# ivanalberico/End-To-End-Self-Supervised-SLAM

Hardware: AMD Instinct MI355X
Metric: online refinement steps/sec @640x480, seq_len=60 (higher is better)
Workload: dtype f32

## Files before the change

end-to-end-self-supervised-slam_amd/csrc/conv.hip:

```cpp
#include <cassert>
#include <type_traits>

#include "e2e_common.h"

typedef float f4v __attribute__((ext_vector_type(4)));
typedef float f16v __attribute__((ext_vector_type(16)));

#define CBK 16

enum { ACT_NONE = 0, ACT_RELU = 1, ACT_ELU = 2, ACT_DISP = 3 };

struct ConvArgs {
    const float* src0;
    const float* src1;
    const float* w;
    const float* scale;
    const float* shift;
    const float* res;
    float* out;
    int B, Hs, Ws;
    int Cin, C1, up;
    int Hd, Wd;
    int Ncols, ldw;
    int KH, KW, stride, pad, pad_mode;
// ... 2046 lines not shown

__global__ __launch_bounds__(256) void k_gather_adjoint(const float* __restrict__ dxp, int B, int Hs, int Ws, int Cin, int C1, int up,
                                                        int pp, float* __restrict__ d0, float* __restrict__ d1, int acc0, int acc1,
                                                        const float* __restrict__ x0, int act0, const float* __restrict__ x1, int act1) {
    const int Hp = Hs + 2 * pp, Wp = Ws + 2 * pp, C2 = Cin - C1, Hl = Hs / up, Wl = Ws / up;
    const int64_t n0 = (int64_t)B * Hl * Wl * C1, n1 = (int64_t)B * Hs * Ws * C2;
    for (int64_t i = (int64_t)blockIdx.x * 256 + threadIdx.x; i < n0 + n1; i += (int64_t)gridDim.x * 256) {
        const bool first = i < n0;
        int64_t t = first ? i : i - n0;
        const int Cx = first ? C1 : C2, Hx = first ? Hl : Hs, Wx = first ? Wl : Ws, u = first ? up : 1;
        const int c = (int)(t % Cx); t /= Cx;
        const int x = (int)(t % Wx); t /= Wx;
        const int y = (int)(t % Hx); t /= Hx;
        const int b = (int)t;
        const int cc = first ? c : C1 + c;
        float s = 0.f;
        for (int dy = 0; dy < u; ++dy)
            for (int dx = 0; dx < u; ++dx) {
                const int fy = y * u + dy, fx = x * u + dx;
                int ys[3] = {fy + pp, -1, -1}, xs[3] = {fx + pp, -1, -1};
                if (pp) {
                    if (fy == 1) ys[1] = 0;
                    if (fy == Hs - 2) ys[2] = Hp - 1;
                    if (fx == 1) xs[1] = 0;
                    if (fx == Ws - 2) xs[2] = Wp - 1;
                }
                for (int iy = 0; iy < 3; ++iy)
                    for (int ix = 0; ix < 3; ++ix)
                        if (ys[iy] >= 0 && xs[ix] >= 0) s += dxp[(((int64_t)b * Hp + ys[iy]) * Wp + xs[ix]) * Cin + cc];
            }
        float* d = first ? d0 + i : d1 + (i - n0);
        const int acc = first ? acc0 : acc1;
        if (first ? act0 : act1) s *= act_deriv(first ? x0[i] : x1[i - n0], first ? act0 : act1);
        *d = acc ? *d + s : s;
    }
}

__global__ __launch_bounds__(256) void k_gather_adjoint4(const float* __restrict__ dxp, int B, int Hs, int Ws, int Cin, int C1, int up,
                                                         int pp, float* __restrict__ d0, float* __restrict__ d1, int acc0, int acc1,
                                                         const float* __restrict__ x0, int act0, const float* __restrict__ x1, int act1) {
    const int Hp = Hs + 2 * pp, Wp = Ws + 2 * pp, C2 = Cin - C1, Hl = Hs / up, Wl = Ws / up;
    const unsigned q0 = (unsigned)B * Hl * Wl * (C1 >> 2), q1 = (unsigned)B * Hs * Ws * (C2 >> 2);
    for (unsigned i = blockIdx.x * 256u + threadIdx.x; i < q0 + q1; i += gridDim.x * 256u) {
        const bool first = i < q0;
        unsigned t = first ? i : i - q0;
        const unsigned Cq = (unsigned)(first ? C1 : C2) >> 2, Hx = first ? Hl : Hs, Wx = first ? Wl : Ws;
        const int u = first ? up : 1;
        const unsigned cq = t % Cq; t /= Cq;
        const unsigned x = t % Wx; t /= Wx;
        const unsigned y = t % Hx;
        const unsigned b = t / Hx;
        const int cc = (first ? 0 : C1) + (int)cq * 4;
        f4v s = {0.f, 0.f, 0.f, 0.f};
        for (int dy = 0; dy < u; ++dy)
            for (int dx = 0; dx < u; ++dx) {
                const int fy = (int)y * u + dy, fx = (int)x * u + dx;
                int ys[3] = {fy + pp, -1, -1}, xs[3] = {fx + pp, -1, -1};
                if (pp) {
                    if (fy == 1) ys[1] = 0;
                    if (fy == Hs - 2) ys[2] = Hp - 1;
                    if (fx == 1) xs[1] = 0;
                    if (fx == Ws - 2) xs[2] = Wp - 1;
                }
#pragma unroll
                for (int iy = 0; iy < 3; ++iy)
#pragma unroll
                    for (int ix = 0; ix < 3; ++ix)
                        if (ys[iy] >= 0 && xs[ix] >= 0) s += *(const f4v*)(dxp + (((int64_t)b * Hp + ys[iy]) * Wp + xs[ix]) * Cin + cc);
            }
        const int64_t e = (int64_t)(first ? i : i - q0) * 4;
        const int act = first ? act0 : act1;
        if (act) {
            const f4v xv = *(const f4v*)((first ? x0 : x1) + e);
#pragma unroll
            for (int k = 0; k < 4; ++k) s[k] *= act_deriv(xv[k], act);
        }
        f4v* d = (f4v*)((first ? d0 : d1) + e);
        if (first ? acc0 : acc1) s += *d;
        *d = s;
    }
}

#define HC 16
__global__ __launch_bounds__(256) void k_head_fwd(const float* __restrict__ x, const float* __restrict__ w ,
                                                  const float* __restrict__ bias, float* __restrict__ y, int B, int H, int W, int act) {
    __shared__ float sw[9 * HC];
    for (int i = threadIdx.x; i < 9 * HC; i += 256) {
        const int ci = i / 9, tap = i - ci * 9;
        sw[tap * HC + ci] = w[i];
    }
    __syncthreads();
    const int64_t N = (int64_t)B * H * W;
    const int q = threadIdx.x & 3;
    for (int64_t n0 = (int64_t)blockIdx.x * 64; n0 < N; n0 += (int64_t)gridDim.x * 64) {
        const int64_t n = n0 + (threadIdx.x >> 2);
        const bool on = n < N;
        const int64_t nn = on ? n : N - 1;
        const int b = (int)(nn / ((int64_t)H * W));
        const int r = (int)(nn - (int64_t)b * H * W), h = r / W, ww = r - h * W;
        float acc = 0.f;
#pragma unroll
        for (int kh = 0; kh < 3; ++kh)
#pragma unroll
            for (int kw = 0; kw < 3; ++kw) {
                const int ys = reflect1(h + kh - 1, H), xs = reflect1(ww + kw - 1, W);
                const f4v v = *(const f4v*)(x + (((int64_t)b * H + ys) * W + xs) * HC + q * 4);
                const float* wt = &sw[(kh * 3 + kw) * HC + q * 4];
                acc = fmaf(v[0], wt[0], fmaf(v[1], wt[1], fmaf(v[2], wt[2], fmaf(v[3], wt[3], acc))));
            }
        acc += __shfl_xor(acc, 1, 64);
        acc += __shfl_xor(acc, 2, 64);
        if (on && q == 0) y[n] = apply_act(acc + (bias ? bias[0] : 0.f), act);
    }
}

__global__ __launch_bounds__(256) void k_head_bwd_data(const float* __restrict__ dz, const float* __restrict__ w, float* __restrict__ dx,
                                                       int B, int H, int W, const float* __restrict__ xin, int dact) {
    __shared__ float sw[9 * HC];
    for (int i = threadIdx.x; i < 9 * HC; i += 256) {
        const int ci = i / 9, tap = i - ci * 9;
        sw[tap * HC + ci] = w[i];
    }
    __syncthreads();
    const int64_t N = (int64_t)B * H * W;
    const int cq = threadIdx.x & 3;
    for (int64_t n = (int64_t)blockIdx.x * 64 + (threadIdx.x >> 2); n < N; n += (int64_t)gridDim.x * 64) {
        const int b = (int)(n / ((int64_t)H * W));
        const int r = (int)(n - (int64_t)b * H * W), h = r / W, ww = r - h * W;
        f4v acc = {0.f, 0.f, 0.f, 0.f};
        const int ry = (h == 1) ? 0 : ((h == H - 2) ? H + 1 : -100);
        const int rx = (ww == 1) ? 0 : ((ww == W - 2) ? W + 1 : -100);
        const float* gz = dz + (int64_t)b * H * W;
#pragma unroll
        for (int kh = 0; kh < 3; ++kh)
#pragma unroll
            for (int kw = 0; kw < 3; ++kw) {
                const float* wt = &sw[(kh * 3 + kw) * HC + cq * 4];
                const int qy0 = h - kh + 1, qx0 = ww - kw + 1, qy1 = ry - kh, qx1 = rx - kw;
                const bool y0 = qy0 >= 0 && qy0 < H, x0 = qx0 >= 0 && qx0 < W, y1 = qy1 >= 0 && qy1 < H, x1 = qx1 >= 0 && qx1 < W;
                float g = (y0 && x0) ? gz[(int64_t)qy0 * W + qx0] : 0.f;
                if (y1 | x1) {
                    if (y0 && x1) g += gz[(int64_t)qy0 * W + qx1];
                    if (y1 && x0) g += gz[(int64_t)qy1 * W + qx0];
                    if (y1 && x1) g += gz[(int64_t)qy1 * W + qx1];
                }
#pragma unroll
                for (int c = 0; c < 4; ++c) acc[c] = fmaf(g, wt[c], acc[c]);
            }
        if (dact) {
            const f4v xv = *(const f4v*)(xin + n * HC + cq * 4);
#pragma unroll
            for (int e = 0; e < 4; ++e) acc[e] *= act_deriv(xv[e], dact);
        }
        *(f4v*)(dx + n * HC + cq * 4) = acc;
    }
}

__global__ __launch_bounds__(256) void k_head_bwd_weight(const float* __restrict__ dz, const float* __restrict__ x, float* __restrict__ partials,
                                                         int B, int H, int W) {
    __shared__ float red[4][9 * HC + 1];
    const int64_t N = (int64_t)B * H * W;
    const int lane = threadIdx.x & 63, wave = threadIdx.x >> 6, cq = threadIdx.x & 3, ps = threadIdx.x >> 2;
    const int64_t per = (N + gridDim.x - 1) / gridDim.x;
    const int64_t n0 = (int64_t)blockIdx.x * per, n1 = (n0 + per < N) ? n0 + per : N;
    float acc[36];
#pragma unroll
    for (int k = 0; k < 36; ++k) acc[k] = 0.f;
    float sb = 0.f;
    for (int64_t n = n0 + ps; n < n1; n += 64) {
        const float g = dz[n];
        const int b = (int)(n / ((int64_t)H * W));
        const int r = (int)(n - (int64_t)b * H * W), h = r / W, ww = r - h * W;
#pragma unroll
        for (int kh = 0; kh < 3; ++kh)
#pragma unroll
            for (int kw = 0; kw < 3; ++kw) {
                const int ys = reflect1(h + kh - 1, H), xs = reflect1(ww + kw - 1, W);
                const f4v v = *(const f4v*)(x + (((int64_t)b * H + ys) * W + xs) * HC + cq * 4);
#pragma unroll
                for (int c = 0; c < 4; ++c) acc[(kh * 3 + kw) * 4 + c] = fmaf(g, v[c], acc[(kh * 3 + kw) * 4 + c]);
            }
        sb += g;
    }
#pragma unroll
    for (int k = 0; k < 36; ++k) {
        float v = acc[k];
#pragma unroll
        for (int o = 4; o < 64; o <<= 1) v += __shfl_xor(v, o, 64);
        acc[k] = v;
    }
#pragma unroll
    for (int o = 4; o < 64; o <<= 1) sb += __shfl_xor(sb, o, 64);
    if (lane < 4) {
#pragma unroll
        for (int t = 0; t < 9; ++t)
#pragma unroll
            for (int c = 0; c < 4; ++c) red[wave][t * HC + lane * 4 + c] = acc[t * 4 + c];
        if (lane == 0) red[wave][9 * HC] = sb;
    }
    __syncthreads();
    if (threadIdx.x < 9 * HC + 1)
        partials[(int64_t)blockIdx.x * (9 * HC + 1) + threadIdx.x] = ((red[0][threadIdx.x] + red[1][threadIdx.x]) + red[2][threadIdx.x]) + red[3][threadIdx.x];
}

__global__ __launch_bounds__(256) void k_head_wreduce(const float* __restrict__ partials, int nparts, float* __restrict__ dw, float* __restrict__ dbias) {
    __shared__ float red[4];
    const int col = blockIdx.x;
    float s = 0.f;
    for (int i = threadIdx.x; i < nparts; i += 256) s += partials[(int64_t)i * (9 * HC + 1) + col];
    const float t = block_sum(s, red);
    if (threadIdx.x == 0) {
        if (col == 9 * HC) { if (dbias) dbias[0] = t; }
        else { const int tap = col / HC, ci = col - tap * HC; dw[ci * 9 + tap] = t; }
    }
}

static inline int egrid(int64_t n) { int64_t g = (n + 255) / 256; return (int)(g < 1 ? 1 : (g > 4096 ? 4096 : g)); }

struct GemmCfg { int bm, bn, S; };
#define WGRAD_TARGET 1024

#define CONV_TILE_SHAPES(X)                                                                                      \
    X(64, 64, 2, 2, 1, 1, 32) X(128, 64, 2, 2, 2, 1, 32) X(128, 128, 2, 2, 2, 2, 16) X(128, 32, 4, 1, 1, 1, 32) \
    X(32, 128, 1, 4, 1, 1, 32) X(32, 64, 1, 2, 1, 1, 32) X(64, 32, 2, 1, 1, 1, 32) X(32, 32, 1, 1, 1, 1, 32)
static int tile_max_cb(int bm, int bn) {
#define X(BM, BN, WM, WN, TM, TN, MAXCB) if (bm == BM && bn == BN) return MAXCB;
    CONV_TILE_SHAPES(X)
// ... 333 lines not shown
    if (rc != E2E_OK) return rc;
    if (!done) launch_gemm<true>(a, 4, workspace, force, (hipStream_t)stream);
    E2E_LAUNCH_CHECK("e2e_conv2d_bwd_data");
    return E2E_OK;
}

int e2e_conv2d_bwd_data(const float* dz, const float* w_bwd, int ld_bwd, float* dxp, int B, int Hs, int Ws, int Cin, int Cout,
                        int Ho, int Wo, int KH, int KW, int stride, int pad, int pad_mode, float* workspace, void* stream) {
    GEOM_BWD_DATA(g);
    return bwd_data_impl(BwdDataOps{dz, w_bwd, ld_bwd, dxp, 0, nullptr, 0, nullptr}, g, workspace, stream);
}

int e2e_conv2d_bwd_data_acc(const float* dz, const float* w_bwd, int ld_bwd, float* dxp, int B, int Hs, int Ws, int Cin, int Cout,
                            int Ho, int Wo, int KH, int KW, int stride, int pad, int pad_mode, int accumulate, float* workspace,
                            void* stream) {
    GEOM_BWD_DATA(g);
    return bwd_data_impl(BwdDataOps{dz, w_bwd, ld_bwd, dxp, accumulate, nullptr, 0, nullptr}, g, workspace, stream);
}

int e2e_conv2d_bwd_data_fused(const float* da, const float* w_bwd, int ld_bwd, float* dxp, int B, int Hs, int Ws, int Cin, int Cout,
                              int Ho, int Wo, int KH, int KW, int stride, int pad, int pad_mode, int accumulate, const float* x_in,
                              int in_act, const float* pre_add, float* workspace, void* stream) {
    GEOM_BWD_DATA(g);
    return bwd_data_impl(BwdDataOps{da, w_bwd, ld_bwd, dxp, accumulate, x_in, in_act, pre_add}, g, workspace, stream);
}

int e2e_conv2d_bwd_data_fused_tuned(const float* da, const float* w_bwd, int ld_bwd, float* dxp, int B, int Hs, int Ws, int Cin, int Cout,
                                    int Ho, int Wo, int KH, int KW, int stride, int pad, int pad_mode, int accumulate, const float* x_in,
                                    int in_act, const float* pre_add, float* workspace, int tile_m, int tile_n, int ksplit, void* stream) {
    E2E_REQUIRE(tuning_ok(tile_m, tile_n, ksplit), E2E_ERR_ARG, "e2e_conv2d_bwd_data_fused_tuned: unsupported decomposition %d x %d / %d", tile_m, tile_n, ksplit);
    GEOM_BWD_DATA(g);
    return bwd_data_impl(BwdDataOps{da, w_bwd, ld_bwd, dxp, accumulate, x_in, in_act, pre_add}, g, workspace, stream, GemmCfg{tile_m, tile_n, ksplit});
}

struct GatherAdjoint { const float* dxp; int B, Hs, Ws, Cin, C1, up, padded; float *d0, *d1; int acc0, acc1; const float* x0; int act0; const float* x1; int act1; };
static void launch_gather_adjoint(const GatherAdjoint& q, hipStream_t st) {
    const int64_t n = (int64_t)q.B * (q.Hs / q.up) * (q.Ws / q.up) * q.C1 + (int64_t)q.B * q.Hs * q.Ws * (q.Cin - q.C1);
    if (q.Cin % 4 == 0 && q.C1 % 4 == 0 && n < (1ll << 31))
        hipLaunchKernelGGL(k_gather_adjoint4, dim3(egrid(n / 4)), dim3(256), 0, st, q.dxp, q.B, q.Hs, q.Ws, q.Cin, q.C1, q.up, q.padded ? 1 : 0, q.d0, q.d1, q.acc0, q.acc1,
                           q.x0, q.act0, q.x1, q.act1);
    else
        hipLaunchKernelGGL(k_gather_adjoint, dim3(egrid(n)), dim3(256), 0, st, q.dxp, q.B, q.Hs, q.Ws, q.Cin, q.C1, q.up, q.padded ? 1 : 0, q.d0, q.d1, q.acc0, q.acc1,
                           q.x0, q.act0, q.x1, q.act1);
}

int e2e_conv2d_gather_adjoint(const float* dxp, int B, int Hs, int Ws, int Cin, int C1, int up, int padded, float* d_src0,
                              float* d_src1, int accumulate0, int accumulate1, void* stream) {
    E2E_REQUIRE(dxp && d_src0 && B > 0 && Cin > 0 && C1 > 0 && C1 <= Cin && (C1 == Cin || d_src1) && (up == 1 || up == 2), E2E_ERR_ARG,
                "e2e_conv2d_gather_adjoint: bad argument");
    launch_gather_adjoint(GatherAdjoint{dxp, B, Hs, Ws, Cin, C1, up, padded, d_src0, d_src1, accumulate0, accumulate1, nullptr, 0, nullptr, 0}, (hipStream_t)stream);
    E2E_LAUNCH_CHECK("e2e_conv2d_gather_adjoint");
    return E2E_OK;
}

int e2e_conv2d_gather_adjoint_act(const float* dxp, int B, int Hs, int Ws, int Cin, int C1, int up, int padded, float* d_src0, float* d_src1,
                                  int accumulate0, int accumulate1, const float* src0, int act0, const float* src1, int act1, void* stream) {
    E2E_REQUIRE(dxp && d_src0 && B > 0 && Cin > 0 && C1 > 0 && C1 <= Cin && (C1 == Cin || d_src1) && (up == 1 || up == 2), E2E_ERR_ARG,
                "e2e_conv2d_gather_adjoint_act: bad argument");
    E2E_REQUIRE((act0 == 0 || src0) && (act1 == 0 || src1) && act0 >= 0 && act0 <= 2 && act1 >= 0 && act1 <= 2, E2E_ERR_ARG,
                "e2e_conv2d_gather_adjoint_act: an activation derivative needs the activation's output");
    launch_gather_adjoint(GatherAdjoint{dxp, B, Hs, Ws, Cin, C1, up, padded, d_src0, d_src1, accumulate0, accumulate1, src0, act0, src1, act1}, (hipStream_t)stream);
    E2E_LAUNCH_CHECK("e2e_conv2d_gather_adjoint_act");
    return E2E_OK;
}

int e2e_conv2d_act_bwd(const float* dy, const float* y, const float* scale, float* dz, int64_t n, int C, int act, void* stream) {
    E2E_REQUIRE(dy && y && dz && n > 0 && C > 0 && act >= 0 && act <= 3, E2E_ERR_ARG, "e2e_conv2d_act_bwd: bad argument");
    hipLaunchKernelGGL(k_act_bwd, dim3(egrid(n)), dim3(256), 0, (hipStream_t)stream, dy, y, scale, dz, n, C, act, 0);
    E2E_LAUNCH_CHECK("e2e_conv2d_act_bwd");
    return E2E_OK;
}

int e2e_conv2d_act_bwd_acc(const float* dy, const float* y, const float* scale, float* dz, int64_t n, int C, int act, int accumulate,
                           void* stream) {
    E2E_REQUIRE(dy && y && dz && n > 0 && C > 0 && act >= 0 && act <= 3, E2E_ERR_ARG, "e2e_conv2d_act_bwd_acc: bad argument");
    hipLaunchKernelGGL(k_act_bwd, dim3(egrid(n)), dim3(256), 0, (hipStream_t)stream, dy, y, scale, dz, n, C, act, accumulate);
    E2E_LAUNCH_CHECK("e2e_conv2d_act_bwd_acc");
    return E2E_OK;
}

#define HEAD_PARTS 2048
int e2e_head_fwd(const float* x, const float* w, const float* bias, float* y, int B, int H, int W, int Cin, int act, void* stream) {
    E2E_REQUIRE(x && w && y && B > 0 && H >= 2 && W >= 2 && Cin == HC, E2E_ERR_ARG, "e2e_head_fwd: bad argument (the head takes %d channels)", HC);
    hipLaunchKernelGGL(k_head_fwd, dim3(egrid((int64_t)B * H * W * 4)), dim3(256), 0, (hipStream_t)stream, x, w, bias, y, B, H, W, act);
    E2E_LAUNCH_CHECK("e2e_head_fwd");
    return E2E_OK;
}
int64_t e2e_head_workspace_floats(void) { return (int64_t)HEAD_PARTS * (9 * HC + 1); }
int e2e_head_bwd_act(const float* dz, const float* x, const float* w, float* dx, float* dw, float* dbias, float* workspace, int B, int H,
                     int W, int Cin, int in_act, void* stream) {
    E2E_REQUIRE(dz && x && w && workspace && B > 0 && H >= 2 && W >= 2 && Cin == HC && in_act >= 0 && in_act <= 2, E2E_ERR_ARG, "e2e_head_bwd: bad argument");
    E2E_REQUIRE((int64_t)B * H * W * HC < (1ll << 31), E2E_ERR_ARG, "e2e_head_bwd: activation too large for 32-bit element offsets");
    hipStream_t st = (hipStream_t)stream;
    if (dx) hipLaunchKernelGGL(k_head_bwd_data, dim3(egrid((int64_t)B * H * W * 4)), dim3(256), 0, st, dz, w, dx, B, H, W, x, in_act);
    if (dw) {
        hipLaunchKernelGGL(k_head_bwd_weight, dim3(HEAD_PARTS), dim3(256), 0, st, dz, x, workspace, B, H, W);
        hipLaunchKernelGGL(k_head_wreduce, dim3(9 * HC + 1), dim3(256), 0, st, workspace, HEAD_PARTS, dw, dbias);
    }
    E2E_LAUNCH_CHECK("e2e_head_bwd");
    return E2E_OK;
}

int e2e_head_bwd(const float* dz, const float* x, const float* w, float* dx, float* dw, float* dbias, float* workspace, int B, int H,
                 int W, int Cin, void* stream) {
    return e2e_head_bwd_act(dz, x, w, dx, dw, dbias, workspace, B, H, W, Cin, 0, stream);
}

enum WgradPath { WP_STEM, WP_THIN, WP_TAPS, WP_GEMM16, WP_GEMM_LEAN, WP_GEMM, WP_COUNT };
struct WgradPlan { WgradPath path; bool open; int64_t S; int Mpad, Npad, tm, tn, nxg, ny, tiles_x, ptx, pty, nchunks, cps; };
#define TAP_TARGET 640
static WgradPlan wgrad_plan(WgradPath path, const ConvGeom& g, int has_bias, bool tuned, int wg_target) {
    const int B = g.B, Ho = g.Ho, Wo = g.Wo, Cin = g.Cin, Cout = g.Cout, KH = g.KH, KW = g.KW;
    WgradPlan p{path};
    if (path == WP_STEM) {
        if (tuned || !(KH == 7 && KW == 7 && Cin == 3 && Cout == 64)) return p;
        p.nxg = ((Wo + 31) / 32 + 1) / 2; p.ny = (Ho + 3) / 4;
        p.S = (int64_t)B * p.ny * p.nxg; p.Mpad = 64; p.Npad = 148;
    } else if (path == WP_THIN) {
        if (tuned || !(KH == 3 && KW == 3 && ((Cout == 16 && (Cin == 16 || Cin == 32)) || (Cout == 32 && Cin == 96)))) return p;
        const int txt = (Wo + 63) / 64;
        p.ny = (Ho + 3) / 4;
        const int64_t total = (int64_t)B * p.ny * txt * (Cin / 16);
        p.tiles_x = 1;
        while (total / p.tiles_x > 1400 && p.tiles_x < txt) ++p.tiles_x;
        p.nxg = (txt + p.tiles_x - 1) / p.tiles_x;
        p.S = (int64_t)B * p.ny * p.nxg; p.Mpad = Cout; p.Npad = (9 * Cin + (has_bias ? 1 : 0) + 3) / 4 * 4;
    } else if (path == WP_TAPS) {
        if (tuned || !(KH == 3 && KW == 3 && Cin % 32 == 0 && Cout % 32 == 0)) return p;
        p.ptx = (Wo + 7) / 8; p.pty = (Ho + 7) / 8;
        p.nchunks = B * p.ptx * p.pty;
        const int tiles = (Cin / 32) * (Cout / 32);
        int S = (TAP_TARGET + tiles - 1) / tiles;
        if (S > p.nchunks) S = p.nchunks;
        if (S < 1) S = 1;
        p.cps = (p.nchunks + S - 1) / S;
        p.S = (p.nchunks + p.cps - 1) / p.cps; p.Mpad = Cout; p.Npad = (9 * Cin + (has_bias ? 1 : 0) + 3) / 4 * 4;
    } else {
        const bool use16 = path == WP_GEMM16;
        if (use16 && Cout != 16) return p;
        const int Ng = KH * KW * Cin + (has_bias ? 1 : 0);
        p.tm = Cout <= 32 ? 32 : 64; p.tn = Cout <= 32 ? 128 : 64;
        if (use16) { p.tm = 16; p.tn = 160; }
        p.Mpad = (Cout + p.tm - 1) / p.tm * p.tm; p.Npad = (Ng + p.tn - 1) / p.tn * p.tn;
        const int64_t P = (int64_t)B * Ho * Wo;
        const int64_t tiles = (int64_t)(p.Mpad / p.tm) * (p.Npad / p.tn);
        const int target = use16 ? wg_target * 3 / 4 : wg_target;
        int64_t S = (target + tiles - 1) / tiles;
        const int64_t maxS = (P + 255) / 256;
        if (S > maxS) S = maxS;
        if (S < 1) S = 1;
        p.S = S;
    }
    p.open = true;
    return p;
}

static int64_t wgrad_workspace_floats(const ConvGeom& g, int has_bias, bool tuned, int wg_target) {
    int64_t n = 0;
    for (int i = 0; i < WP_COUNT; ++i) {
        const WgradPlan p = wgrad_plan((WgradPath)i, g, has_bias, tuned, wg_target);
        if (p.open && p.S * p.Mpad * p.Npad > n) n = p.S * p.Mpad * p.Npad;
    }
    return n;
}

static WgradPlan wgrad_choose(const ConvGeom& g, int has_bias, bool has_src1, bool tuned, int wg_target) {
    const int Hs = g.Hs, Ws = g.Ws, Cin = g.Cin, Cout = g.Cout, Ho = g.Ho, Wo = g.Wo, stride = g.stride, pad = g.pad, pad_mode = g.pad_mode, C1 = g.C1, up = g.up;
    const int vec = (Cin % 4 == 0 && C1 % 4 == 0) ? 4 : 1;
    const int64_t P = (int64_t)g.B * Ho * Wo;
    auto plan = [&](WgradPath w) { return wgrad_plan(w, g, has_bias, tuned, wg_target); };
    const bool lean = vec == 4 && Cout % 4 == 0 && Wo >= 8 && (int64_t)g.B * Hs * Ws * Cin * 4 < (1ll << 31) && P * Cout * 4 < (1ll << 31) && P < (1ll << 24);
    WgradPlan p{WP_GEMM};
    if (stride == 2 && pad == 3 && pad_mode == 0 && C1 == Cin && up == 1 && !has_bias && Ho == (Hs + 6 - 7) / 2 + 1 && Wo == (Ws + 6 - 7) / 2 + 1 &&
        (p = plan(WP_STEM)).open)
        return p;
    if (lean && stride == 1 && pad == 1 && pad_mode == 1 && C1 % 16 == 0 && Ho == Hs && Wo == Ws && (C1 == Cin || has_src1) && Hs % up == 0 && Ws % up == 0 &&
        (p = plan(WP_THIN)).open)
// ... 211 lines not shown
```

end-to-end-self-supervised-slam_amd/csrc/depth_ops.hip:

```cpp
#include "e2e_common.h"

#define DT 256

__device__ __forceinline__ unsigned int f2key(float f) {
    const unsigned int b = __float_as_uint(f);
    return (b & 0x80000000u) ? ~b : (b | 0x80000000u);
}
__device__ __forceinline__ float key2f(unsigned int k) {
    return __uint_as_float((k & 0x80000000u) ? (k & 0x7FFFFFFFu) : ~k);
}

#define MED_BINS 2048
struct MedState {
    unsigned int prefix, rank, key, index, count;
};

__device__ unsigned int select_bin(const unsigned int* __restrict__ hist, int nb, unsigned int r, unsigned int* r_in, unsigned int* sh) {
    unsigned int c[8], s = 0;
#pragma unroll
    for (int j = 0; j < 8; ++j) {
        const int i = threadIdx.x * 8 + j;
        c[j] = (i < nb) ? hist[i] : 0u;
        s += c[j];
    }
    unsigned int x = s;
#pragma unroll
    for (int o = 1; o < 64; o <<= 1) {
        const unsigned int y = __shfl_up(x, o, 64);
        if ((threadIdx.x & 63) >= o) x += y;
    }
    __syncthreads();
    if ((threadIdx.x & 63) == 63) sh[2 + (threadIdx.x >> 6)] = x;
    __syncthreads();
    unsigned int woff = 0;
    for (int w = 0; w < (int)(threadIdx.x >> 6); ++w) woff += sh[2 + w];
    const unsigned int excl = woff + x - s;
    if (r >= excl && r < excl + s) {
        unsigned int acc = excl;
#pragma unroll
        for (int j = 0; j < 8; ++j) {
            if (r < acc + c[j]) { sh[0] = threadIdx.x * 8 + j; sh[1] = r - acc; break; }
            acc += c[j];
        }
    }
    __syncthreads();
    *r_in = sh[1];
    return sh[0];
}

template <int PASS, bool RECIP = false>
__global__ __launch_bounds__(DT) void k_median_hist(const float* __restrict__ x, int64_t n, unsigned int rank0,
                                                    unsigned int* __restrict__ hist , MedState* __restrict__ st,
                                                    float* __restrict__ recip_out = nullptr) {
    __shared__ unsigned int lh[MED_BINS];
    __shared__ unsigned int sh[8];
    for (int i = threadIdx.x; i < MED_BINS; i += DT) lh[i] = 0;
    unsigned int prefix = 0;
    if (PASS == 1) {
        unsigned int rin;
        const unsigned int b = select_bin(hist, MED_BINS, rank0, &rin, sh);
        prefix = b << 21;
        if (blockIdx.x == 0 && threadIdx.x == 0) { st->prefix = prefix; st->rank = rin; }
    } else if (PASS == 2) {
        unsigned int rin0, rin1;
        const unsigned int b0 = select_bin(hist, MED_BINS, rank0, &rin0, sh);
        __syncthreads();
        const unsigned int b1 = select_bin(hist + MED_BINS, MED_BINS, rin0, &rin1, sh);
        prefix = (b0 << 21) | (b1 << 10);
        if (blockIdx.x == 0 && threadIdx.x == 0) { st->prefix = prefix; st->rank = rin1; }
    }
    __syncthreads();
    for (int64_t i = (int64_t)blockIdx.x * DT + threadIdx.x; i < n; i += (int64_t)gridDim.x * DT) {
        float v = x[i];
        if (RECIP) { v = 1.0f / v; recip_out[i] = v; }
        const unsigned int k = f2key(v);
        if (PASS == 0) atomicAdd(&lh[k >> 21], 1u);
        else if (PASS == 1) { if ((k >> 21) == (prefix >> 21)) atomicAdd(&lh[(k >> 10) & 2047u], 1u); }
        else { if ((k >> 10) == (prefix >> 10)) atomicAdd(&lh[k & 1023u], 1u); }
    }
    __syncthreads();
    unsigned int* gh = hist + PASS * MED_BINS;
    for (int i = threadIdx.x; i < MED_BINS; i += DT)
        if (lh[i]) atomicAdd(&gh[i], lh[i]);
}

__global__ __launch_bounds__(DT) void k_median_final(const float* __restrict__ x, int64_t n, const unsigned int* __restrict__ hist,
                                                     MedState* __restrict__ st, float* __restrict__ value_out) {
    __shared__ unsigned int sh[8];
    unsigned int rin;
    const unsigned int b2 = select_bin(hist + 2 * MED_BINS, 1024, st->rank, &rin, sh);
    const unsigned int key = st->prefix | b2;
    if (blockIdx.x == 0 && threadIdx.x == 0) { st->key = key; *value_out = key2f(key); }
    for (int64_t i = (int64_t)blockIdx.x * DT + threadIdx.x; i < n; i += (int64_t)gridDim.x * DT)
        if (f2key(x[i]) == key) { atomicMin(&st->index, (unsigned int)i); atomicAdd(&st->count, 1u); }
}

__global__ __launch_bounds__(DT) void k_median_final_scale(const float* __restrict__ delta, int64_t n, const unsigned int* __restrict__ hist,
                                                           MedState* __restrict__ st, const float* __restrict__ m_gt, float* __restrict__ median_out,
                                                           float* __restrict__ depth, float* __restrict__ ratio_out) {
    __shared__ unsigned int sh[8];
    unsigned int rin;
    const unsigned int b2 = select_bin(hist + 2 * MED_BINS, 1024, st->rank, &rin, sh);
    const unsigned int key = st->prefix | b2;
    const float med = key2f(key);
    const float rho = m_gt[0] / med;
    if (blockIdx.x == 0 && threadIdx.x == 0) {
        st->key = key;
        *median_out = med;
        if (ratio_out) ratio_out[0] = rho;
    }
    for (int64_t i = (int64_t)blockIdx.x * DT + threadIdx.x; i < n; i += (int64_t)gridDim.x * DT) {
        const float d = delta[i];
        depth[i] = d * rho;
        if (f2key(d) == key) { atomicMin(&st->index, (unsigned int)i); atomicAdd(&st->count, 1u); }
    }
}

__global__ void k_median_init(unsigned int* hist, MedState* st) {
    for (int i = threadIdx.x; i < 3 * MED_BINS; i += blockDim.x) hist[i] = 0;
    if (threadIdx.x == 0) { st->prefix = 0; st->rank = 0; st->key = 0; st->index = 0xFFFFFFFFu; st->count = 0; }
}

__global__ __launch_bounds__(DT) void k_dot_partials(const float* __restrict__ a, const float* __restrict__ b, int64_t n,
                                                     float* __restrict__ partials) {
    __shared__ float red[DT / 64];
    float acc = 0.f;
    for (int64_t i = (int64_t)blockIdx.x * DT + threadIdx.x; i < n; i += (int64_t)gridDim.x * DT) acc = fmaf(a[i], b[i], acc);
    const float s = block_sum(acc, red);
    if (threadIdx.x == 0) partials[blockIdx.x] = s;
}

__global__ __launch_bounds__(DT) void k_scale_chain_bwd(const float* __restrict__ g, const float* __restrict__ delta,
                                                        const float* __restrict__ m_gt, const float* __restrict__ m_delta,
                                                        const MedState* __restrict__ st, const float* __restrict__ partials,
                                                        int nparts, float* __restrict__ g_disp, int64_t n, const int* __restrict__ elems, int n_elems) {
    __shared__ float sS;
    if (threadIdx.x == 0) {
        double acc = 0.0;
        for (int i = 0; i < nparts; ++i) acc += (double)partials[i];
        sS = (float)acc;
    }
    __syncthreads();
    const float md = m_delta[0], rho = m_gt[0] / md;
    const float corr = -(rho / md) * sS;
    const float share = corr / (float)(n_elems > 0 ? (unsigned int)n_elems : st->count);
    for (int64_t i = (int64_t)blockIdx.x * DT + threadIdx.x; i < n; i += (int64_t)gridDim.x * DT) {
        const float d = delta[i];
        float gd = rho * g[i];
        if (n_elems > 0) {
            for (int e = 0; e < n_elems; ++e) if ((int)i == elems[e]) gd += share;
        } else if (d == md) gd += share;
        g_disp[i] = -(d * d) * gd;
    }
}

__global__ __launch_bounds__(DT) void k_diff_partials(const float* __restrict__ a, const float* __restrict__ b, int64_t n, int kind,
                                                      float* __restrict__ partials) {
    __shared__ float red[DT / 64];
    float acc = 0.f;
    for (int64_t i = (int64_t)blockIdx.x * DT + threadIdx.x; i < n; i += (int64_t)gridDim.x * DT) {
        const float e = a[i] - b[i];
        acc += (kind == 2) ? e * e : fabsf(e);
    }
    const float s = block_sum(acc, red);
    if (threadIdx.x == 0) partials[blockIdx.x] = s;
}

__global__ void k_sum_partials(const float* __restrict__ partials, int nparts, double scale, float* __restrict__ out) {
    __shared__ double sh[4];
    double acc = 0.0;
    for (int i = threadIdx.x; i < nparts; i += blockDim.x) acc += (double)partials[i];
    acc = wave_sum_d(acc);
    if ((threadIdx.x & 63) == 0) sh[threadIdx.x >> 6] = acc;
    __syncthreads();
    if (threadIdx.x == 0) out[0] = (float)((((sh[0] + sh[1]) + sh[2]) + sh[3]) * scale);
}

__global__ __launch_bounds__(DT) void k_diff_bwd(const float* __restrict__ a, const float* __restrict__ b, const float* __restrict__ g,
                                                 int64_t n, int kind, float* __restrict__ gb) {
    const float s = g[0] / (float)n;
    for (int64_t i = (int64_t)blockIdx.x * DT + threadIdx.x; i < n; i += (int64_t)gridDim.x * DT) {
        const float e = a[i] - b[i];
        gb[i] = (kind == 2) ? s * (-2.f * e) : s * ((e > 0.f) ? -1.f : ((e < 0.f) ? 1.f : 0.f));
    }
}

#define NMET 8
__global__ __launch_bounds__(DT) void k_metrics_partials(const float* __restrict__ gt, const float* __restrict__ pred, int64_t n,
                                                         int mask_zero_gt, float* __restrict__ partials) {
    __shared__ float red[DT / 64];
    float acc[NMET] = {0.f, 0.f, 0.f, 0.f, 0.f, 0.f, 0.f, 0.f};
    for (int64_t i = (int64_t)blockIdx.x * DT + threadIdx.x; i < n; i += (int64_t)gridDim.x * DT) {
        const float g = gt[i], p = pred[i];
        if (mask_zero_gt && g == 0.f) continue;
        const float th = fmaxf(g / p, p / g);
        const float e = g - p, le = logf(g) - logf(p);
        acc[0] += fabsf(e) / g;
        acc[1] += (e * e) / g;
        acc[2] += e * e;
        acc[3] += le * le;
        acc[4] += (th < 1.25f) ? 1.f : 0.f;
        acc[5] += (th < 1.5625f) ? 1.f : 0.f;
        acc[6] += (th < 1.953125f) ? 1.f : 0.f;
        acc[7] += 1.f;
    }
    for (int m = 0; m < NMET; ++m) {
        const float s = block_sum(acc[m], red);
        if (threadIdx.x == 0) partials[m * gridDim.x + blockIdx.x] = s;
        __syncthreads();
    }
}

__global__ void k_metrics_final(const float* __restrict__ partials, int nparts, float* __restrict__ out) {
    __shared__ double tot[NMET];
    if (threadIdx.x < NMET) {
        double acc = 0.0;
        for (int i = 0; i < nparts; ++i) acc += (double)partials[threadIdx.x * nparts + i];
        tot[threadIdx.x] = acc;
    }
    __syncthreads();
    if (threadIdx.x < 7) {
        double v = tot[threadIdx.x] / tot[7];
        if (threadIdx.x == 2 || threadIdx.x == 3) v = sqrt(v);
        out[threadIdx.x] = (float)v;
    }
}

__global__ __launch_bounds__(DT) void k_adam(float* __restrict__ p, const float* __restrict__ g, float* __restrict__ m, float* __restrict__ v,
                                             int64_t n, float one_minus_b1, float b2, float one_minus_b2, float step_size,
                                             float bc2_sqrt, float eps, const float* __restrict__ participants,
                                             const float2* __restrict__ schedule, const int* __restrict__ step_counter, int schedule_len) {
    const int64_t n4 = n >> 2;
    const float cnt = participants ? fmaxf(participants[0], 1.f) : 1.f;
    if (schedule) {
        int t = step_counter[0];
        t = t < 1 ? 1 : (t > schedule_len ? schedule_len : t);
        const float2 sc = schedule[t - 1];
        step_size = sc.x;
        bc2_sqrt = sc.y;
    }
    float4* p4 = (float4*)p; const float4* g4 = (const float4*)g; float4* m4 = (float4*)m; float4* v4 = (float4*)v;
    for (int64_t i = (int64_t)blockIdx.x * DT + threadIdx.x; i < n4; i += (int64_t)gridDim.x * DT) {
        float4 pp = p4[i], gg = g4[i], mm = m4[i], vv = v4[i];
        float* pa = (float*)&pp; float* ga = (float*)&gg; float* ma = (float*)&mm; float* va = (float*)&vv;
#pragma unroll
        for (int k = 0; k < 4; ++k) {
            ga[k] = ga[k] / cnt;
            ma[k] = ma[k] + one_minus_b1 * (ga[k] - ma[k]);
            va[k] = va[k] * b2 + one_minus_b2 * (ga[k] * ga[k]);
            const float den = sqrtf(va[k]) / bc2_sqrt + eps;
            pa[k] = pa[k] - step_size * (ma[k] / den);
        }
        p4[i] = pp; m4[i] = mm; v4[i] = vv;
    }
    for (int64_t i = (n4 << 2) + (int64_t)blockIdx.x * DT + threadIdx.x; i < n; i += (int64_t)gridDim.x * DT) {
        const float gi = g[i] / cnt;
        const float mi = m[i] + one_minus_b1 * (gi - m[i]);
        const float vi = v[i] * b2 + one_minus_b2 * (gi * gi);
        m[i] = mi; v[i] = vi;
        p[i] = p[i] - step_size * (mi / (sqrtf(vi) / bc2_sqrt + eps));
    }
}

__global__ void k_adam_advance(int* __restrict__ step_counter) { step_counter[0] += 1; }

static inline int sgrid(int64_t n, int cap = 1024) {
    int64_t g = (n + DT - 1) / DT;
    return (int)(g < 1 ? 1 : (g > cap ? cap : g));
}
#define RED_PARTS 512

extern "C" {

int64_t e2e_median_workspace_bytes(void) { return (3 * MED_BINS + 8) * 4; }

int e2e_median_lower(const float* x, int64_t n, float* value_out, void* workspace, void* stream) {
    E2E_REQUIRE(n > 0 && n < 0xFFFFFFFFll && x && value_out && workspace, E2E_ERR_ARG, "e2e_median_lower: bad argument");
    hipStream_t st = (hipStream_t)stream;
    unsigned int* hist = (unsigned int*)workspace;
    MedState* ms = (MedState*)(hist + 3 * MED_BINS);
    const unsigned int rank = (unsigned int)((n - 1) / 2);
    const int g = sgrid(n, 96);
    hipLaunchKernelGGL(k_median_init, dim3(1), dim3(256), 0, st, hist, ms);
    hipLaunchKernelGGL(k_median_hist<0>, dim3(g), dim3(DT), 0, st, x, n, rank, hist, ms, (float*)nullptr);
    hipLaunchKernelGGL(k_median_hist<1>, dim3(g), dim3(DT), 0, st, x, n, rank, hist, ms, (float*)nullptr);
    hipLaunchKernelGGL(k_median_hist<2>, dim3(g), dim3(DT), 0, st, x, n, rank, hist, ms, (float*)nullptr);
    hipLaunchKernelGGL(k_median_final, dim3(g), dim3(DT), 0, st, x, n, hist, ms, value_out);
    E2E_LAUNCH_CHECK("e2e_median_lower");
    return E2E_OK;
}

int64_t e2e_depth_scale_workspace_bytes(void) { return e2e_median_workspace_bytes() + RED_PARTS * 4 + 64; }

int e2e_depth_scale_fwd(const float* disp, const float* median_gt, float* delta, float* depth, float* median_delta,
                        float* ratio_out, void* workspace, int64_t n, void* stream) {
    E2E_REQUIRE(n > 0 && disp && median_gt && delta && depth && median_delta && workspace, E2E_ERR_ARG, "e2e_depth_scale_fwd: bad argument");
    hipStream_t st = (hipStream_t)stream;
    E2E_REQUIRE(n < 0xFFFFFFFFll, E2E_ERR_ARG, "e2e_depth_scale_fwd: too many elements");
    unsigned int* hist = (unsigned int*)workspace;
    MedState* ms = (MedState*)(hist + 3 * MED_BINS);
    const unsigned int rank = (unsigned int)((n - 1) / 2);
    const int g = sgrid(n, 96);
    hipLaunchKernelGGL(k_median_init, dim3(1), dim3(256), 0, st, hist, ms);
    hipLaunchKernelGGL((k_median_hist<0, true>), dim3(g), dim3(DT), 0, st, disp, n, rank, hist, ms, delta);
    hipLaunchKernelGGL(k_median_hist<1>, dim3(g), dim3(DT), 0, st, (const float*)delta, n, rank, hist, ms, (float*)nullptr);
    hipLaunchKernelGGL(k_median_hist<2>, dim3(g), dim3(DT), 0, st, (const float*)delta, n, rank, hist, ms, (float*)nullptr);
    hipLaunchKernelGGL(k_median_final_scale, dim3(sgrid(n)), dim3(DT), 0, st, (const float*)delta, n, (const unsigned int*)hist, ms, median_gt, median_delta, depth, ratio_out);
    E2E_LAUNCH_CHECK("e2e_depth_scale_fwd");
    return E2E_OK;
}

__global__ __launch_bounds__(DT) void k_fixed_scale_fwd(const float* __restrict__ disp, float scale, float* __restrict__ delta, float* __restrict__ depth,
                                                        int64_t n) {
    for (int64_t i = (int64_t)blockIdx.x * DT + threadIdx.x; i < n; i += (int64_t)gridDim.x * DT) {
        const float d = 1.f / disp[i];
        if (delta) delta[i] = d;
        depth[i] = d * scale;
    }
}
__global__ __launch_bounds__(DT) void k_fixed_scale_bwd(const float* __restrict__ g_depth, const float* __restrict__ disp, float scale,
                                                        float* __restrict__ g_disp, int64_t n) {
    for (int64_t i = (int64_t)blockIdx.x * DT + threadIdx.x; i < n; i += (int64_t)gridDim.x * DT) {
        const float d = 1.f / disp[i];
        g_disp[i] = -(g_depth[i] * scale) * d * d;
    }
}

int e2e_depth_fixed_scale_fwd(const float* disp, float scale, float* delta, float* depth, int64_t n, void* stream) {
    E2E_REQUIRE(n > 0 && disp && depth, E2E_ERR_ARG, "e2e_depth_fixed_scale_fwd: bad argument");
    hipLaunchKernelGGL(k_fixed_scale_fwd, dim3(sgrid(n)), dim3(DT), 0, (hipStream_t)stream, disp, scale, delta, depth, n);
    E2E_LAUNCH_CHECK("e2e_depth_fixed_scale_fwd");
    return E2E_OK;
}

int e2e_depth_fixed_scale_bwd(const float* g_depth, const float* disp, float scale, float* g_disp, int64_t n, void* stream) {
    E2E_REQUIRE(n > 0 && g_depth && disp && g_disp, E2E_ERR_ARG, "e2e_depth_fixed_scale_bwd: bad argument");
    hipLaunchKernelGGL(k_fixed_scale_bwd, dim3(sgrid(n)), dim3(DT), 0, (hipStream_t)stream, g_depth, disp, scale, g_disp, n);
    E2E_LAUNCH_CHECK("e2e_depth_fixed_scale_bwd");
    return E2E_OK;
}

int e2e_depth_scale_bwd(const float* g_depth, const float* delta, const float* median_gt, const float* median_delta,
                        float* g_disp, void* workspace, int64_t n, void* stream) {
    return e2e_depth_scale_bwd_at(g_depth, delta, median_gt, median_delta, nullptr, 0, g_disp, workspace, n, stream);
}

int e2e_depth_scale_bwd_at(const float* g_depth, const float* delta, const float* median_gt, const float* median_delta, const int* elements,
                           int n_elements, float* g_disp, void* workspace, int64_t n, void* stream) {
    E2E_REQUIRE(n > 0 && g_depth && delta && median_gt && median_delta && g_disp && workspace, E2E_ERR_ARG, "e2e_depth_scale_bwd: bad argument");
    E2E_REQUIRE(n_elements >= 0 && n_elements <= 64 && (n_elements == 0 || elements), E2E_ERR_ARG, "e2e_depth_scale_bwd_at: 0..64 named elements");
    hipStream_t st = (hipStream_t)stream;
    const MedState* ms = (const MedState*)((unsigned int*)workspace + 3 * MED_BINS);
    float* parts = (float*)((char*)workspace + e2e_median_workspace_bytes() + 32);
// ... 79 lines not shown
```

Baseline: 215.6.

## Tile head forward conv through shared memory and stage scale-chain partials

```diff
diff --git a/end-to-end-self-supervised-slam_amd/csrc/conv.hip b/end-to-end-self-supervised-slam_amd/csrc/conv.hip
--- a/end-to-end-self-supervised-slam_amd/csrc/conv.hip
+++ b/end-to-end-self-supervised-slam_amd/csrc/conv.hip
@@ -2152,38 +2152,48 @@
 }
 
 #define HC 16
+#define HT_H 4
+#define HT_W 64
 __global__ __launch_bounds__(256) void k_head_fwd(const float* __restrict__ x, const float* __restrict__ w ,
                                                   const float* __restrict__ bias, float* __restrict__ y, int B, int H, int W, int act) {
     __shared__ float sw[9 * HC];
+    __shared__ f4v sx[(HT_H + 2) * (HT_W + 2) * (HC / 4)];
     for (int i = threadIdx.x; i < 9 * HC; i += 256) {
         const int ci = i / 9, tap = i - ci * 9;
         sw[tap * HC + ci] = w[i];
     }
-    __syncthreads();
-    const int64_t N = (int64_t)B * H * W;
-    const int q = threadIdx.x & 3;
-    for (int64_t n0 = (int64_t)blockIdx.x * 64; n0 < N; n0 += (int64_t)gridDim.x * 64) {
-        const int64_t n = n0 + (threadIdx.x >> 2);
-        const bool on = n < N;
-        const int64_t nn = on ? n : N - 1;
-        const int b = (int)(nn / ((int64_t)H * W));
-        const int r = (int)(nn - (int64_t)b * H * W), h = r / W, ww = r - h * W;
-        float acc = 0.f;
-#pragma unroll
-        for (int kh = 0; kh < 3; ++kh)
-#pragma unroll
-            for (int kw = 0; kw < 3; ++kw) {
-                const int ys = reflect1(h + kh - 1, H), xs = reflect1(ww + kw - 1, W);
-                const f4v v = *(const f4v*)(x + (((int64_t)b * H + ys) * W + xs) * HC + q * 4);
-                const float* wt = &sw[(kh * 3 + kw) * HC + q * 4];
-                acc = fmaf(v[0], wt[0], fmaf(v[1], wt[1], fmaf(v[2], wt[2], fmaf(v[3], wt[3], acc))));
-            }
-        acc += __shfl_xor(acc, 1, 64);
-        acc += __shfl_xor(acc, 2, 64);
-        if (on && q == 0) y[n] = apply_act(acc + (bias ? bias[0] : 0.f), act);
-    }
-}
-
+    const int tx = (W + HT_W - 1) / HT_W, ty = (H + HT_H - 1) / HT_H;
+    const int64_t ntiles = (int64_t)B * ty * tx;
+    const int q = threadIdx.x & 3, col = threadIdx.x >> 2;
+    for (int64_t t = blockIdx.x; t < ntiles; t += gridDim.x) {
+        const int b = (int)(t / ((int64_t)ty * tx));
+        const int r = (int)(t - (int64_t)b * ty * tx), y0 = (r / tx) * HT_H, x0 = (r % tx) * HT_W;
+        __syncthreads();
+        for (int i = threadIdx.x; i < (HT_H + 2) * (HT_W + 2) * 4; i += 256) {
+            const int p = i >> 2, sr = p / (HT_W + 2), sc = p - sr * (HT_W + 2);
+            const int ys = y0 - 1 + sr, xs = x0 - 1 + sc;
+            if (ys <= H && xs <= W) sx[i] = *(const f4v*)(x + (((int64_t)b * H + reflect1(ys, H)) * W + reflect1(xs, W)) * HC + (i & 3) * 4);
+        }
+        __syncthreads();
+#pragma unroll
+        for (int j = 0; j < HT_H; ++j) {
+            float acc = 0.f;
+#pragma unroll
+            for (int kh = 0; kh < 3; ++kh)
+#pragma unroll
+                for (int kw = 0; kw < 3; ++kw) {
+                    const f4v v = sx[((j + kh) * (HT_W + 2) + col + kw) * 4 + q];
+                    const float* wt = &sw[(kh * 3 + kw) * HC + q * 4];
+                    acc = fmaf(v[0], wt[0], fmaf(v[1], wt[1], fmaf(v[2], wt[2], fmaf(v[3], wt[3], acc))));
+                }
+            acc += __shfl_xor(acc, 1, 64);
+            acc += __shfl_xor(acc, 2, 64);
+            if (q == 0 && y0 + j < H && x0 + col < W) y[((int64_t)b * H + y0 + j) * W + x0 + col] = apply_act(acc + (bias ? bias[0] : 0.f), act);
+        }
+    }
+}
+
+template <bool N3>
 __global__ __launch_bounds__(256) void k_head_bwd_data(const float* __restrict__ dz, const float* __restrict__ w, float* __restrict__ dx,
                                                        int B, int H, int W, const float* __restrict__ xin, int dact) {
     __shared__ float sw[9 * HC];
@@ -2200,6 +2210,7 @@
         f4v acc = {0.f, 0.f, 0.f, 0.f};
         const int ry = (h == 1) ? 0 : ((h == H - 2) ? H + 1 : -100);
         const int rx = (ww == 1) ? 0 : ((ww == W - 2) ? W + 1 : -100);
+        const int ry2 = (N3 && H == 3 && h == 1) ? H + 1 : -100, rx2 = (N3 && W == 3 && ww == 1) ? W + 1 : -100;
         const float* gz = dz + (int64_t)b * H * W;
 #pragma unroll
         for (int kh = 0; kh < 3; ++kh)
@@ -2213,6 +2224,15 @@
                     if (y0 && x1) g += gz[(int64_t)qy0 * W + qx1];
                     if (y1 && x0) g += gz[(int64_t)qy1 * W + qx0];
                     if (y1 && x1) g += gz[(int64_t)qy1 * W + qx1];
+                }
+                if (N3) {
+                    const int qy2 = ry2 - kh, qx2 = rx2 - kw;
+                    const bool y2 = qy2 >= 0 && qy2 < H, x2 = qx2 >= 0 && qx2 < W;
+                    if (y0 && x2) g += gz[(int64_t)qy0 * W + qx2];
+                    if (y1 && x2) g += gz[(int64_t)qy1 * W + qx2];
+                    if (y2 && x0) g += gz[(int64_t)qy2 * W + qx0];
+                    if (y2 && x1) g += gz[(int64_t)qy2 * W + qx1];
+                    if (y2 && x2) g += gz[(int64_t)qy2 * W + qx2];
                 }
 #pragma unroll
                 for (int c = 0; c < 4; ++c) acc[c] = fmaf(g, wt[c], acc[c]);
@@ -2712,7 +2732,8 @@
 #define HEAD_PARTS 2048
 int e2e_head_fwd(const float* x, const float* w, const float* bias, float* y, int B, int H, int W, int Cin, int act, void* stream) {
     E2E_REQUIRE(x && w && y && B > 0 && H >= 2 && W >= 2 && Cin == HC, E2E_ERR_ARG, "e2e_head_fwd: bad argument (the head takes %d channels)", HC);
-    hipLaunchKernelGGL(k_head_fwd, dim3(egrid((int64_t)B * H * W * 4)), dim3(256), 0, (hipStream_t)stream, x, w, bias, y, B, H, W, act);
+    const int64_t tiles = (int64_t)B * ((H + HT_H - 1) / HT_H) * ((W + HT_W - 1) / HT_W);
+    hipLaunchKernelGGL(k_head_fwd, dim3((unsigned)(tiles < 65536 ? tiles : 65536)), dim3(256), 0, (hipStream_t)stream, x, w, bias, y, B, H, W, act);
     E2E_LAUNCH_CHECK("e2e_head_fwd");
     return E2E_OK;
 }
@@ -2722,7 +2743,8 @@
     E2E_REQUIRE(dz && x && w && workspace && B > 0 && H >= 2 && W >= 2 && Cin == HC && in_act >= 0 && in_act <= 2, E2E_ERR_ARG, "e2e_head_bwd: bad argument");
     E2E_REQUIRE((int64_t)B * H * W * HC < (1ll << 31), E2E_ERR_ARG, "e2e_head_bwd: activation too large for 32-bit element offsets");
     hipStream_t st = (hipStream_t)stream;
-    if (dx) hipLaunchKernelGGL(k_head_bwd_data, dim3(egrid((int64_t)B * H * W * 4)), dim3(256), 0, st, dz, w, dx, B, H, W, x, in_act);
+    if (dx && (H == 3 || W == 3)) hipLaunchKernelGGL(k_head_bwd_data<true>, dim3(egrid((int64_t)B * H * W * 4)), dim3(256), 0, st, dz, w, dx, B, H, W, x, in_act);
+    else if (dx) hipLaunchKernelGGL(k_head_bwd_data<false>, dim3(egrid((int64_t)B * H * W * 4)), dim3(256), 0, st, dz, w, dx, B, H, W, x, in_act);
     if (dw) {
         hipLaunchKernelGGL(k_head_bwd_weight, dim3(HEAD_PARTS), dim3(256), 0, st, dz, x, workspace, B, H, W);
         hipLaunchKernelGGL(k_head_wreduce, dim3(9 * HC + 1), dim3(256), 0, st, workspace, HEAD_PARTS, dw, dbias);
diff --git a/end-to-end-self-supervised-slam_amd/csrc/depth_ops.hip b/end-to-end-self-supervised-slam_amd/csrc/depth_ops.hip
--- a/end-to-end-self-supervised-slam_amd/csrc/depth_ops.hip
+++ b/end-to-end-self-supervised-slam_amd/csrc/depth_ops.hip
@@ -1,6 +1,7 @@
 #include "e2e_common.h"
 
 #define DT 256
+#define RED_PARTS 512
 
 __device__ __forceinline__ unsigned int f2key(float f) {
     const unsigned int b = __float_as_uint(f);
@@ -134,10 +135,14 @@
                                                         const float* __restrict__ m_gt, const float* __restrict__ m_delta,
                                                         const MedState* __restrict__ st, const float* __restrict__ partials,
                                                         int nparts, float* __restrict__ g_disp, int64_t n, const int* __restrict__ elems, int n_elems) {
+    __shared__ float sp[RED_PARTS];
     __shared__ float sS;
+    for (int i = threadIdx.x; i < nparts; i += DT) sp[i] = partials[i];
+    __syncthreads();
     if (threadIdx.x == 0) {
         double acc = 0.0;
-        for (int i = 0; i < nparts; ++i) acc += (double)partials[i];
+#pragma unroll 8
+        for (int i = 0; i < nparts; ++i) acc += (double)sp[i];
         sS = (float)acc;
     }
     __syncthreads();
@@ -268,7 +273,6 @@
     int64_t g = (n + DT - 1) / DT;
     return (int)(g < 1 ? 1 : (g > cap ? cap : g));
 }
-#define RED_PARTS 512
 
 extern "C" {
 
```

New measurement: 216.7 (median of 6 runs). No clear change (+0.5%).
